# thelovelab/DESeq2

Hardware: AMD Instinct MI355X
Metric: genes/sec for DESeq() disp+beta+Wald fit, 50k x 500 x p=4 (throughput of steps pipelined two deep; one call at a time: one_call_at_a_time) (higher is better)
Workload: dtype f64; 1 GPU; BASELINE configs[2]: 50k genes x 500 samples, ~batch+condition (p=4), Wald; 50000 non-zero genes in total, sharded over 1 GPU(s) in the contiguous ranges of R/parallel.R:10; inputs resident in HBM in R layout (int32 counts, f64 nf matrix; the fused chain reads the size factors as the m-vector the matrix was built from); genes_total=50000, genes_this_gpu=50000, samples=500, p=4, test=Wald, parallelism=gene-shard x1, chain=fused device-driven (dsq_deseq_dev), steps_overlap=step k enqueued while step k-1's results are copied and post-processed

## Files before the change

deseq2_amd/csrc/aux.hip:

```cpp
#include "dsq_internal.hpp"
#include "dsq_math.hpp"
#include "dsq_wave.hpp"

namespace dsq {

static constexpr int kAuxBatch = 4;

static inline int aux_grid_fwd(int n) {
    int blocks = (n + 3) / 4;
    int cap = device_cu_count() * 8;
    return blocks < cap ? (blocks < 1 ? 1 : blocks) : cap;
}

static constexpr int kTileS = 256;
__host__ __device__ static inline bool aux_tiled(int m, int p) { return (size_t)m * p >= 8192 && p <= 24; }

template <int P, bool USE_W, bool TILED>
__global__ void __launch_bounds__(256) prefit_kernel(PrefitKernelParams kp) {
    extern __shared__ __attribute__((aligned(16))) double tile[];
    const int lane = threadIdx.x & 63;
    const int wave = threadIdx.x >> 6;
    const int waves = blockDim.x >> 6;
    const int m = kp.m;
    double rr[P][P];
#pragma unroll
    for (int c = 0; c < P; c++)
#pragma unroll
        for (int k = 0; k < P; k++) rr[c][k] = kp.r[c + P * k];
    const int nwork = DSQ_NWORK(kp);
    for (int wbase = blockIdx.x * waves; wbase < nwork; wbase += gridDim.x * waves) {
        const int wi = wbase + wave;
        const bool active = wi < nwork;
        if (!TILED && !active) break;
        const int g = DSQ_GENE(kp, active ? wi : nwork - 1);
        const int32_t *yg = kp.y + (size_t)g * kp.ld;
        const double *nfg = kp.nf_is_vector ? kp.nf : kp.nf + (size_t)g * kp.ld;
        const double *wg = USE_W ? kp.weights + (size_t)g * kp.ld : nullptr;
        int32_t yb[kAuxBatch];
        double nb[kAuxBatch], wb[kAuxBatch];
        auto load_row = [&](int j, int b) {
            yb[b] = yg[j]; nb[b] = nfg[j];
            if constexpr (USE_W) wb[b] = wg[j];
        };
        double a2[2] = {0.0, 0.0};
        sweep_batched<kAuxBatch>(m, lane, load_row, [&](int, int b) {
            double yy = (double)yb[b];
            double cn = yy / nb[b];
            if constexpr (USE_W) cn = wb[b] * cn;
            a2[0] += cn;
            a2[1] += yy;
        });
        wave_allreduce_many(a2, lane);
        const double mean = a2[0] / (double)m;
        double av = 0.0;
        sweep_batched<kAuxBatch>(m, lane, load_row, [&](int, int b) {
            double cn = (double)yb[b] / nb[b];
            if constexpr (USE_W) cn = wb[b] * cn;
            double dlt = cn - mean;
            av += dlt * dlt;
        });
        av = wave_allreduce(av);
        double tu[2 * P];
#pragma unroll
        for (int c = 0; c < 2 * P; c++) tu[c] = 0.0;
        double ae = 0.0;
        if constexpr (TILED) {
            static_assert(kTileS == 64 * kAuxBatch, "one tile = one batch of trips");
            auto stage = [&](const double *src, int t0) {
                __syncthreads();
                const int ts = (m - t0) < kTileS ? (m - t0) : kTileS;
                for (int idx = threadIdx.x; idx < P * kTileS; idx += blockDim.x) {
                    const int c = idx / kTileS, jj = idx - c * kTileS;
                    if (jj < ts) tile[idx] = src[(size_t)c * m + t0 + jj];
                }
                __syncthreads();
            };
            for (int t0 = 0; t0 < m; t0 += kTileS) {
                stage(kp.q, t0);
                _Pragma("unroll")
                for (int b = 0; b < kAuxBatch; b++) { const int j = t0 + 64 * b + lane; if (j < m) { yb[b] = yg[j]; nb[b] = nfg[j]; } }
                _Pragma("unroll")
                for (int b = 0; b < kAuxBatch; b++) {
                    const int j = t0 + 64 * b + lane;
                    if (j < m) {
                        double yn = (double)yb[b] / nb[b];
                        double ly = dlog(yn + 0.1);
#pragma unroll
                        for (int c = 0; c < P; c++) {
                            double qv = tile[c * kTileS + 64 * b + lane];
// ... 645 lines not shown
hipError_t launch_trend_fit_dev_zeroed(const double *means, const double *disps, const int32_t *n_dev, double *coefs,
                                       int32_t *status, void *workspace, hipStream_t st) {
    hipLaunchKernelGGL(trend_fit_kernel, dim3(kTrendBlocks), dim3(1024), 0, st, means, disps, 0L, n_dev, coefs, status,
                       (TrendWs *)workspace);
    return hipGetLastError();
}

static inline int aux_grid(int n) {
    int blocks = (n + 3) / 4;
    int cap = device_cu_count() * 8;
    return blocks < cap ? (blocks < 1 ? 1 : blocks) : cap;
}

template <int P>
static hipError_t launch_prefit_p(const PrefitKernelParams &kp, hipStream_t st) {
    if constexpr (P <= 24) {
        if (aux_tiled(kp.m, P)) {
            const size_t lds = (size_t)P * kTileS * sizeof(double);
            if (kp.useWeights) hipLaunchKernelGGL((prefit_kernel<P, true, true>), dim3(aux_grid(kp.n)), dim3(256), lds, st, kp);
            else hipLaunchKernelGGL((prefit_kernel<P, false, true>), dim3(aux_grid(kp.n)), dim3(256), lds, st, kp);
            return hipGetLastError();
        }
    }
    if (kp.useWeights) hipLaunchKernelGGL((prefit_kernel<P, true, false>), dim3(aux_grid(kp.n)), dim3(256), 0, st, kp);
    else hipLaunchKernelGGL((prefit_kernel<P, false, false>), dim3(aux_grid(kp.n)), dim3(256), 0, st, kp);
    return hipGetLastError();
}

hipError_t launch_prefit(const PrefitKernelParams &kp, hipStream_t st, bool *ok) {
    *ok = true;
    switch (kp.p) {
#define DSQ_X(W) case W: return launch_prefit_p<W>(kp, st);
    DSQ_P_EACH(DSQ_X)
#undef DSQ_X
    default: *ok = false; return hipSuccess;
    }
}

template <int P>
static hipError_t launch_linear_mu_p(const PrefitKernelParams &kp, double mu_floor, double *mu, hipStream_t st) {
    if constexpr (P <= 24) {
        if (aux_tiled(kp.m, P)) {
            hipLaunchKernelGGL((linear_mu_kernel<P, true>), dim3(aux_grid(kp.n)), dim3(256), (size_t)P * kTileS * sizeof(double), st, kp, mu_floor, mu);
            return hipGetLastError();
        }
    }
// ... 36 lines not shown
```

deseq2_amd/csrc/pipeline.hip:

```cpp
#include "capi.hpp"
#include "dsq_math.hpp"
#include "dsq_wave.hpp"

#include <algorithm>
#include <cstdio>
#include <cstdlib>
#include <cstring>
#include <vector>

namespace dsq {

hipError_t launch_trend_fit_dev(const double *means, const double *disps, const int32_t *n_dev, double *coefs,
                                int32_t *status, void *workspace, hipStream_t st);
hipError_t launch_trend_fit_dev_zeroed(const double *means, const double *disps, const int32_t *n_dev, double *coefs,
                                       int32_t *status, void *workspace, hipStream_t st);
size_t trend_fit_workspace_bytes();

DSQ_DEV double np_min(double a, double b) { return (a != a || b != b) ? a + b : (a < b ? a : b); }
DSQ_DEV double np_max(double a, double b) { return (a != a || b != b) ? a + b : (a > b ? a : b); }

struct Rows {
    const int32_t *rows;
    const int32_t *n_dev;
    int n;
};
DSQ_DEV int rows_count(const Rows &r) { return r.n_dev ? *r.n_dev : r.n; }
DSQ_DEV int rows_gene(const Rows &r, int i) { return r.rows ? r.rows[i] : i; }

__global__ void __launch_bounds__(1024) compact_kernel(int mode, int n, int32_t *allZero, const int32_t *force_zero,
                                                       const double *mean_in, const double *disp_in, double thresh,
                                                       int32_t *rows_out, double *mean_out, double *disp_out,
                                                       int32_t *count_out) {
    constexpr int NT = 4;
    __shared__ int wcnt[NT][16];
    __shared__ int base_s;
    const int t = threadIdx.x, lane = t & 63, wave = t >> 6;
    if (t == 0) base_s = 0;
    __syncthreads();
    for (int i0 = 0; i0 < n; i0 += NT * 1024) {
        bool keep[NT];
        double mv[NT], dv[NT];
#pragma unroll
        for (int q = 0; q < NT; q++) {
            const int i = i0 + q * 1024 + t;
            keep[q] = false; mv[q] = 0.0; dv[q] = 0.0;
            if (i < n) {
                if (mode == 0) {
                    int z = allZero[i] | (force_zero ? force_zero[i] : 0);
                    if (force_zero) allZero[i] = z ? 1 : 0;
                    keep[q] = !z;
                } else {
                    dv[q] = disp_in[i]; mv[q] = mean_in[i];
                    keep[q] = dv[q] > thresh;
                }
            }
        }
        unsigned long long mask[NT];
#pragma unroll
        for (int q = 0; q < NT; q++) {
            mask[q] = __ballot(keep[q]);
            if (lane == 0) wcnt[q][wave] = __popcll(mask[q]);
        }
        __syncthreads();
        int off = base_s;
#pragma unroll
        for (int q = 0; q < NT; q++) {
            int mine = off;
            for (int w = 0; w < 16; w++) { const int c = wcnt[q][w]; if (w < wave) mine += c; off += c; }
            mine += __popcll(mask[q] & ((1ull << lane) - 1ull));
            if (keep[q]) {
                const int i = i0 + q * 1024 + t;
                if (mode == 0) rows_out[mine] = i;
                else { mean_out[mine] = mv[q]; disp_out[mine] = dv[q]; }
            }
        }
        __syncthreads();
        if (t == 0) base_s = off;
        __syncthreads();
    }
    if (t == 0) *count_out = base_s;
}

DSQ_DEV uint64_t key_of(double d) {
    uint64_t u = d2bits(d);
    return (u >> 63) ? ~u : (u | 0x8000000000000000ULL);
}
DSQ_DEV double double_of(uint64_t k) {
    uint64_t u = (k >> 63) ? (k & 0x7fffffffffffffffULL) : ~k;
    return bits2d(u);
}

static constexpr int kSelDirect = 1024;
DSQ_DEV uint64_t rank_direct(const uint64_t *keys, int cnt, long rank, unsigned long long *bc) {
    for (int t = threadIdx.x; t < cnt; t += blockDim.x) {
        const uint64_t mine = keys[t];
        int before = 0;
        for (int j = 0; j < cnt; j++) {
            const uint64_t o = keys[j];
            before += (o < mine || (o == mine && j < t)) ? 1 : 0;
        }
        if (before == (int)rank) bc[0] = mine;
    }
    __syncthreads();
// ... 426 lines not shown
    double minDisp, maxDisp, xim, outlierSD;
    const double *xim_dev;
    int maxit, betaMaxit;
    const double *baseMean, *baseVar, *roughDisp;
    double *alpha_init, *la0;
    const double *la_out, *initial_lp, *last_lp;
    const int32_t *iter;
    const double *la_grid;
    double *dge;
    int32_t *dispGeneIter;
    int32_t *grid_flag, *grid_rows, *grid_count;
    const double *scalars;
    double *dispFit, *log_dfit, *la_init, *dispMAP, *dispersion;
    const double *dispFit_in;
    int32_t *dispIter, *dispOutlier;
    const double *beta_nat, *beta_var, *beta_iter, *logLike;
    double *beta, *betaSE, *stat, *pvalue, *betaIter_out;
    int32_t *betaConv, *optim_flag, *optim_count;
    int32_t *optim_rows;
    int wald;
    const double *beta_init;
    double *opt_start;
    const int32_t *opt_conv;
};

__global__ void alpha_init_kernel(RuleParams q) {
    const int i = blockIdx.x * blockDim.x + threadIdx.x;
    if (i >= rows_count(q.rw)) return;
    const int g = rows_gene(q.rw, i);
    const double bm = q.baseMean[g], bv = q.baseVar[g];
    const double xim = q.xim_dev ? *q.xim_dev : q.xim;
    const double mom = (bv - xim * bm) / (bm * bm);
    double a = np_min(q.roughDisp[g], mom);
    a = np_min(np_max(q.minDisp, a), q.maxDisp);
    q.alpha_init[g] = a;
    q.la0[g] = dlog(a);
}

__global__ void gene_est_post_kernel(RuleParams q) {
    const int i = blockIdx.x * blockDim.x + threadIdx.x;
    if (i >= rows_count(q.rw)) return;
    const int g = rows_gene(q.rw, i);
    double d = np_min(dexp(q.la_out[g]), q.maxDisp);
    const double ilp = q.initial_lp[g];
    if (q.last_lp[g] < ilp + __builtin_fabs(ilp) / 1e6) d = q.alpha_init[g];
    const int it = q.iter[g];
    q.dispGeneIter[g] = it;
    const bool conv = (it < q.maxit) && !(it == 1);
    const bool refit = !conv && (d > q.minDisp * 10.0);
    q.dge[g] = d;
    q.grid_flag[g] = refit ? 1 : 0;
    if (refit) q.grid_rows[atomicAdd(q.grid_count, 1)] = g;
}

__global__ void gene_est_final_kernel(RuleParams q) {
    const int i = blockIdx.x * blockDim.x + threadIdx.x;
    if (i >= rows_count(q.rw)) return;
    const int g = rows_gene(q.rw, i);
    double d = q.dge[g];
    if (q.grid_flag[g]) d = dexp(q.la_grid[g]);
    q.dge[g] = np_min(np_max(d, q.minDisp), q.maxDisp);
}

__global__ void map_init_kernel(RuleParams q) {
    const int i = blockIdx.x * blockDim.x + threadIdx.x;
    if (i >= rows_count(q.rw)) return;
    const int g = rows_gene(q.rw, i);
    const double fit = q.dispFit_in ? q.dispFit_in[g] : q.scalars[DSQ_SC_COEF0] + q.scalars[DSQ_SC_COEF1] / q.baseMean[g];
    const double d = q.dge[g];
    double init = (d > 0.1 * fit) ? d : fit;
    if (init != init) init = fit;
    q.dispFit[g] = fit;
    q.log_dfit[g] = dlog(fit);
    q.la_init[g] = dlog(init);
}

__global__ void map_post_kernel(RuleParams q) {
    const int i = blockIdx.x * blockDim.x + threadIdx.x;
    if (i >= rows_count(q.rw)) return;
    const int g = rows_gene(q.rw, i);
    const int it = q.iter[g];
    q.dispMAP[g] = dexp(q.la_out[g]);
    q.dispIter[g] = it;
    const bool refit = !(it < q.maxit);
    q.grid_flag[g] = refit ? 1 : 0;
    if (refit) q.grid_rows[atomicAdd(q.grid_count, 1)] = g;
}

__global__ void map_final_kernel(RuleParams q) {
    const int i = blockIdx.x * blockDim.x + threadIdx.x;
    if (i >= rows_count(q.rw)) return;
    const int g = rows_gene(q.rw, i);
// ... 48 lines not shown
    }
}

__global__ void optim_post_kernel(RuleParams q) {
    const int cnt = rows_count(q.rw);
    for (int i = blockIdx.x * blockDim.x + threadIdx.x; i < cnt; i += gridDim.x * blockDim.x) {
        const int g = rows_gene(q.rw, i);
        if (q.betaConv && q.opt_conv[g]) q.betaConv[g] = 1;
        if (q.wald && q.stat) {
            for (int c = 0; c < q.p; c++) {
                const double z = q.beta[(size_t)g + (size_t)q.n * c] / q.betaSE[(size_t)g + (size_t)q.n * c];
                q.stat[(size_t)g + (size_t)q.n * c] = z;
                q.pvalue[(size_t)g + (size_t)q.n * c] = dpnorm_upper2(z);
            }
        }
    }
}

__global__ void list_kernel(Rows rw, const int32_t *flag, int want, int32_t *rows_out, int32_t *count) {
    const int i = blockIdx.x * blockDim.x + threadIdx.x;
    if (i >= rows_count(rw)) return;
    const int g = rows_gene(rw, i);
    if ((flag[g] != 0) == (want != 0)) rows_out[atomicAdd(count, 1)] = g;
}

struct NaRowsParams {
    Rows rw;
    int n, p;
    const int32_t *allZero, *n_refit;
    double *beta, *betaSE, *stat, *pvalue, *betaIter, *logLike, *logLikeReduced, *maxCooks;
    int32_t *betaConv;
};
__global__ void na_rows_kernel(NaRowsParams q) {
    const int i = blockIdx.x * blockDim.x + threadIdx.x;
    if (i >= rows_count(q.rw) || *q.n_refit <= 0) return;
    const int g = rows_gene(q.rw, i);
    if (!q.allZero[g]) return;
    const double nan = dnan();
    for (int c = 0; c < q.p; c++) {
        q.beta[(size_t)g + (size_t)q.n * c] = nan;
        q.betaSE[(size_t)g + (size_t)q.n * c] = nan;
        if (q.stat) { q.stat[(size_t)g + (size_t)q.n * c] = nan; q.pvalue[(size_t)g + (size_t)q.n * c] = nan; }
    }
    q.betaIter[g] = nan; q.logLike[g] = nan; q.maxCooks[g] = nan;
    if (q.logLikeReduced) q.logLikeReduced[g] = nan;
    q.betaConv[g] = -1;
// ... 176 lines not shown
    memset(&kp, 0, sizeof kp);
    kp.n = P.n; kp.m = P.m; kp.ld = P.ld;
    kp.y = y; kp.nf = P.a->nf; kp.nf_is_vector = P.a->nf_is_vector;
    kp.weights = P.a->useWeights ? weights : nullptr; kp.useWeights = kp.weights ? 1 : 0;
    kp.rows = rw.rows; kp.n_dev = rw.n_dev;
    return kp;
}

static RuleParams rule_params(const Pipe &P, const Rows &rw) {
    RuleParams q;
    memset(&q, 0, sizeof q);
    const DsqDeseqArgs *a = P.a;
    const DsqDeseqOut *o = P.o;
    q.rw = rw; q.n = P.n; q.p = P.p;
    q.minDisp = a->minDisp; q.maxDisp = P.maxDisp; q.xim = a->xim; q.outlierSD = a->outlierSD;
    q.xim_dev = a->nf_is_vector ? nullptr : P.xim_cur;
    q.maxit = a->maxit; q.betaMaxit = P.t_maxit;
    q.baseMean = o->baseMean; q.baseVar = o->baseVar; q.roughDisp = P.roughDisp;
    q.alpha_init = P.alpha_init; q.la0 = P.la0;
    q.la_out = P.la_out; q.initial_lp = P.initial_lp; q.last_lp = P.last_lp; q.iter = P.iter; q.la_grid = P.la_grid;
    q.dge = o->dispGeneEst; q.dispGeneIter = o->dispGeneIter;
    q.grid_flag = P.grid_flag; q.grid_rows = P.rows_grid;
    q.scalars = o->scalars;
    q.dispFit_in = a->dispFit_in;
    q.dispFit = o->dispFit; q.log_dfit = P.log_dfit; q.la_init = P.la_init; q.dispMAP = o->dispMAP;
    q.dispersion = o->dispersion; q.dispIter = o->dispIter; q.dispOutlier = o->dispOutlier;
    q.beta_nat = P.beta_nat; q.beta_var = P.beta_var; q.beta_iter = P.beta_iter;
    q.optim_rows = P.rows_opt; q.beta_init = P.beta_init; q.opt_start = P.opt_start; q.opt_conv = P.opt_conv;
    return q;
}

enum { DES_FULL = 0, DES_REDUCED = 1, DES_PRIOR = 2 };
struct DesignSel {
    const double *x, *beta_init, *lam;
    int p;
    const int32_t *cperm, *cstart;
    int ncell;
    int p_true;
};
static DesignSel design_of(const Pipe &P, int which) {
    const DsqDeseqArgs *a = P.a;
    DesignSel d;
    if (which == DES_REDUCED) d = {P.red_x_k, P.red_binit, P.red_lam, P.red_pk, P.red_cell_perm, P.red_cell_start, P.red_ncell, a->p_red};
    else if (which == DES_PRIOR) d = {P.pri_x_k, a->prior_expanded ? P.red_binit : P.beta_init, P.lam_prior, P.pri_pk,
                                      P.cell_perm, P.cell_start, P.ncell, a->p_prior};
    else d = {P.x_k, P.beta_init, P.lam, P.pk, P.cell_perm, P.cell_start, P.ncell, P.p};
    return d;
// ... 117 lines not shown
    kp.beta = via_work ? P.opt_beta : beta; kp.betaSE = via_work ? P.opt_se : betaSE;
    kp.conv = P.opt_conv; kp.mu_out = mu_out; kp.loglike = loglike;
    bool ok = false;
    char nm[32];
    snprintf(nm, sizeof nm, "optim_rows%s", P.tag);
    capi_prof_begin(nm, P.n, P.st);
    DSQ_HIP(dispatch_optim_rows(kp.p, kp, P.st, &ok));
    capi_prof_end(P.st);
    if (!ok) return capi_fail(DSQ_ERR_UNSUPPORTED, "dsq_deseq_dev: no optim kernel for p=%d", P.p);
    if (via_work) {
        hipLaunchKernelGGL(copy_rows_cols_kernel, dim3(16), dim3(256), 0, P.st, orw, P.n, ds.p_true, (const double *)P.opt_beta,
                           (const double *)P.opt_se, beta, betaSE);
        DSQ_HIP(hipGetLastError());
    }
    return DSQ_OK;
}

static Rows lpt_rows(Pipe &P, const Rows &rw, const int32_t *key_i, const double *key_d, int small_first = 0) {
    if (!tuning().lpt || rw.rows != P.rows_nz || P.n > tuning().lpt_maxn) return rw;
    hipLaunchKernelGGL(lpt_order_kernel, dim3(1), dim3(1024), 0, P.st, rw, key_i, key_d, small_first, P.rows_lpt);
    return Rows{P.rows_lpt, rw.n_dev, rw.n};
}

static int gene_est(Pipe &P, const Rows &rw, const int32_t *y, double *mu_hat, int cnt_grid, int cnt_optim,
                    int32_t *optim_flag) {
    const DsqDeseqArgs *a = P.a;
    RuleParams q = rule_params(P, rw);
    hipLaunchKernelGGL(alpha_init_kernel, ew_grid(P.n), dim3(256), 0, P.st, q);
    int rc;
    if (a->linearMu) {
        bool ok = false;
        capi_prof_begin("linear_mu", P.n, P.st);
        DSQ_HIP(launch_linear_mu(prefit_params(P, rw, y), P.ge_floor, mu_hat, P.st, &ok));
        capi_prof_end(P.st);
        if (!ok) return capi_fail(DSQ_ERR_UNSUPPORTED, "dsq_deseq_dev: p=%d", P.p);
    } else {
        rc = launch_fit_beta(P, lpt_rows(P, rw, nullptr, P.o->baseMean, 1), y, P.alpha_init, a->weights_norm, mu_hat, P.ge_floor, nullptr,
                             1e-8, 100, 1, 0.5, "fit_beta");
        if (rc) return rc;
        RuleParams b = rule_params(P, rw);
        b.betaMaxit = 100;
        b.optim_flag = optim_flag; b.optim_count = P.counters + cnt_optim;
        hipLaunchKernelGGL(beta_post_kernel, ew_grid(P.n), dim3(256), 0, P.st, b);
        rc = launch_optim(P, cnt_optim, y, P.alpha_init, a->weights_norm, 0.5, P.ge_floor, P.opt_beta, P.opt_se, P.opt_ll, mu_hat);
        if (rc) return rc;
    }
    rc = launch_fit_disp(P, rw, y, mu_hat, P.la0, P.la0, false, a->weights_floor, a->useCR != 0, false, "fit_disp");
    if (rc) return rc;
    q.grid_count = P.counters + cnt_grid;
    hipLaunchKernelGGL(gene_est_post_kernel, ew_grid(P.n), dim3(256), 0, P.st, q);
    Rows gr = {P.rows_grid, P.counters + cnt_grid, P.n};
    rc = launch_fit_disp(P, gr, y, mu_hat, P.la0, P.la0, false, a->weights_floor, a->useCR != 0, true, "fit_disp_grid");
    if (rc) return rc;
    hipLaunchKernelGGL(gene_est_final_kernel, ew_grid(P.n), dim3(256), 0, P.st, q);
    DSQ_HIP(hipGetLastError());
    return DSQ_OK;
}

static int map_est(Pipe &P, const Rows &rw, const int32_t *y, const double *mu_hat, int cnt_grid) {
    const DsqDeseqArgs *a = P.a;
    RuleParams q = rule_params(P, rw);
    hipLaunchKernelGGL(map_init_kernel, ew_grid(P.n), dim3(256), 0, P.st, q);
    int rc = launch_fit_disp(P, rw, y, mu_hat, P.la_init, P.log_dfit, true, a->weights_norm, a->useCR != 0, false, "fit_disp");
    if (rc) return rc;
    q.grid_count = P.counters + cnt_grid;
    hipLaunchKernelGGL(map_post_kernel, ew_grid(P.n), dim3(256), 0, P.st, q);
    Rows gr = {P.rows_grid, P.counters + cnt_grid, P.n};
    rc = launch_fit_disp(P, gr, y, mu_hat, P.la_init, P.log_dfit, true, a->weights_norm, true, true, "fit_disp_grid");
    if (rc) return rc;
    hipLaunchKernelGGL(map_final_kernel, ew_grid(P.n), dim3(256), 0, P.st, q);
    DSQ_HIP(hipGetLastError());
    return DSQ_OK;
}

__global__ void prior_start_kernel(Rows rw, int n, int p, int intercept, const double *bm, double *binit) {
    const int i = blockIdx.x * blockDim.x + threadIdx.x;
    if (i >= rows_count(rw)) return;
    const int g = rows_gene(rw, i);
    for (int c = 0; c < p; c++) binit[(size_t)g + (size_t)n * c] = intercept ? (c == 0 ? dlog(bm[g]) : 0.0) : 1.0;
}

static int mle_fit(Pipe &P, const Rows &rw, const int32_t *y, double *mu_out, double *hat) {
    const DsqDeseqArgs *a = P.a;
    const DsqDeseqOut *o = P.o;
// ... 378 lines not shown
    }
    P.pri_x_k = a->x_prior; P.pri_pk = P.pkp;
    if (a->betaPrior && P.pkp > a->p_prior)
        if ((rc = capi_pad_design(DSQ_WS_PIPE_PADXR, a->x_prior, m, a->p_prior, P.pkp, st, &P.pri_x_k))) return rc;
    if (a->cell_of && a->ncell > 0)
        P.ncell = capi_upload_cells(a->cell_of, m, DSQ_WS_PIPE_CELLS, st, &P.cell_perm, &P.cell_start);
    if (a->x_red || a->betaPrior) {
        if (a->x_red && a->cell_of_red && a->ncell_red > 0)
            P.red_ncell = capi_upload_cells(a->cell_of_red, m, DSQ_WS_PIPE_CELLS_RED, st, &P.red_cell_perm, &P.red_cell_start);
        void *b;
        if ((rc = capi_ws_get(DSQ_WS_PIPE_RED_MU, (size_t)n * P.ld * sizeof(double), &b))) return rc;
        P.red_mu = (double *)b;
    }
    return DSQ_OK;
}

static int xim_scratch(const Pipe &P, double **out) {
    void *b;
    const int rc = capi_ws_get(DSQ_WS_PIPE_XIM_SCRATCH, ((size_t)P.m + 8) * sizeof(double), &b);
    *out = (double *)b;
    return rc;
}

static int phase_gene_est(Pipe &P, const Rows &nz) {
    const DsqDeseqArgs *a = P.a;
    const DsqDeseqOut *o = P.o;
    const Rows all = {nullptr, nullptr, P.n};
    int rc = launch_prefit_rows(P, all, a->y);
    if (rc) return rc;
    hipLaunchKernelGGL(compact_kernel, dim3(1), dim3(1024), 0, P.st, 0, P.n, o->allZero, a->force_zero,
                       (const double *)nullptr, (const double *)nullptr, 0.0, P.rows_nz, (double *)nullptr,
                       (double *)nullptr, P.counters + CNT_NZ);
    if (!a->nf_is_vector) {
        double *b;
        if ((rc = xim_scratch(P, &b))) return rc;
        DSQ_HIP(launch_xim_rows(a->nf, P.rows_nz, P.counters + CNT_NZ, P.m, P.ld, b, P.xim_dev, P.st));
    }
    return gene_est(P, nz, a->y, o->mu_hat, CNT_GRID1, CNT_OPT1, o->optim_geneest);
}

static int phase_trend(Pipe &P) {
    const DsqDeseqArgs *a = P.a;
    const DsqDeseqOut *o = P.o;
    hipStream_t st = P.st;
    const double *tm = a->trend_mean ? a->trend_mean : o->baseMean;
    const double *td = a->trend_mean ? a->trend_disp : o->dispGeneEst;
    const int nt = a->trend_mean ? a->n_trend : P.n;
    if (!(a->phases & DSQ_PH_GENE_EST)) DSQ_HIP(hipMemsetAsync(P.counters + CNT_TREND, 0, sizeof(int32_t), st));
    hipLaunchKernelGGL(compact_kernel, dim3(1), dim3(1024), 0, st, 1, nt, (int32_t *)nullptr, (const int32_t *)nullptr,
                       tm, td, 100.0 * a->minDisp, (int32_t *)nullptr, P.trend_mean_c, P.trend_disp_c,
                       P.counters + CNT_TREND);
    capi_prof_begin("trend_fit", nt, st);
    if (a->dispFit_in) {
        hipLaunchKernelGGL(trend_given_kernel, dim3(1), dim3(1), 0, st, o->scalars, o->status);
    } else {
        if (a->fitType != DSQ_FIT_MEAN)
            DSQ_HIP(launch_trend_fit_dev_zeroed(P.trend_mean_c, P.trend_disp_c, P.counters + CNT_TREND, o->scalars + DSQ_SC_COEF0,
                                                 o->status + DSQ_ST_TREND_STATUS, P.trend_ws, st));
        if (a->fitType != DSQ_FIT_PARAMETRIC)
            hipLaunchKernelGGL(trend_mean_kernel, dim3(1), dim3(1024), 0, st, td, nt, a->minDisp, (int)a->fitType, o->scalars, o->status);
    }
    capi_prof_end(st);
    capi_prof_begin("prior_var", nt, st);
    const double *fin = a->dispFit_in ? (a->trend_mean ? a->trend_fit_in : a->dispFit_in) : (const double *)nullptr;
    if (!P.sel_ws)
        hipLaunchKernelGGL(prior_var_kernel, dim3(1), dim3(1024), 0, st, tm, td, nt, a->minDisp, a->expVarLogDisp,
                           (P.m > P.p) ? 1 : 0, P.resbuf, o->scalars, o->status, fin, a->dispPriorVar_in);
    else
        hipLaunchKernelGGL(prior_var_grid_kernel, dim3(kSelBlocks), dim3(1024), 0, st, tm, td, nt, a->minDisp, a->expVarLogDisp,
                           (P.m > P.p) ? 1 : 0, P.resbuf, o->scalars, o->status, fin, a->dispPriorVar_in, (SelWs *)P.sel_ws);
    capi_prof_end(st);
    DSQ_HIP(hipGetLastError());
    return DSQ_OK;
}

static int phase_map_test(Pipe &P, const Rows &nz, bool *counters_zeroed) {
    const DsqDeseqArgs *a = P.a;
    const DsqDeseqOut *o = P.o;
    if (!(a->phases & DSQ_PH_GENE_EST)) {
        DSQ_HIP(hipMemsetAsync(P.counters + CNT_GRID2, 0, sizeof(int32_t), P.st));
        DSQ_HIP(hipMemsetAsync(P.counters + CNT_OPT2, 0, sizeof(int32_t), P.st));
        DSQ_HIP(hipMemsetAsync(P.counters + CNT_OPT3, 0, sizeof(int32_t), P.st));
    }
    int rc = map_est(P, nz, a->y, o->mu_hat, CNT_GRID2);
    if (rc) return rc;
    if ((rc = test_fit(P, nz, a->y, o->mu, o->H, CNT_OPT2))) return rc;
    const bool z = *counters_zeroed = (a->phases & (DSQ_PH_OUTLIERS | DSQ_PH_OUTLIERS_DETECT)) && !((a->phases & DSQ_PH_PRIOR) && a->betaPrior);
    hipLaunchKernelGGL(na_assay_rows_kernel, ew_grid(P.n), dim3(256), 0, P.st, P.n, P.m, P.ld, (const int32_t *)o->allZero, o->mu, o->H,
                       z ? P.counters + CNT_REP : (int32_t *)nullptr, z ? (int)(CNT_N - CNT_REP) : 0);
    return DSQ_OK;
}

static int phase_prior(Pipe &P, const Rows &nz) {
    DSQ_HIP(hipMemsetAsync(P.counters + CNT_OPT2, 0, sizeof(int32_t), P.st));
    return prior_fit(P, nz, P.a->y, CNT_OPT2);
}

static int phase_outlier_detect(Pipe &P, const Rows &nz, const OutlierMeta &M, bool counters_zeroed) {
    const DsqDeseqArgs *a = P.a;
    const DsqDeseqOut *o = P.o;
    const int n = P.n, m = P.m;
    hipStream_t st = P.st;
    if (!counters_zeroed) DSQ_HIP(hipMemsetAsync(P.counters + CNT_REP, 0, (CNT_N - CNT_REP) * sizeof(int32_t), st));
    CooksKernelParams ck;
    memset(&ck, 0, sizeof ck);
    ck.n = n; ck.m = m; ck.p = P.p; ck.ld = P.ld; ck.y = a->y; ck.nf = a->nf; ck.nf_is_vector = a->nf_is_vector;
    ck.mu = o->mu; ck.H = o->H; ck.perm = M.dperm; ck.cell_start = M.dstart; ck.in3 = M.din3; ck.ncell = a->ncell; ck.any3 = M.any3;
// ... 5 lines not shown
    capi_prof_begin("cooks_distance", n, st);
    DSQ_HIP(launch_cooks(ck, st, &ok));
    capi_prof_end(st);
    if (!ok) return capi_fail(DSQ_ERR_UNSUPPORTED, "m=%d samples: a gene row plus its sort buffer exceeds the 160 KiB LDS", m);
    hipLaunchKernelGGL(na_assay_rows_kernel, ew_grid(n), dim3(256), 0, st, n, m, P.ld, (const int32_t *)o->allZero, o->cooks,
                       (double *)nullptr);
    if (!a->do_replace) return DSQ_OK;
    ReplaceKernelParams rk;
    memset(&rk, 0, sizeof rk);
    rk.n = n; rk.m = m; rk.ld = P.ld; rk.y = a->y; rk.nf = a->nf; rk.nf_is_vector = a->nf_is_vector;
    rk.cooks = o->cooks; rk.cutoff = a->cooksCutoff; rk.trim = a->trim; rk.replaceable = M.drepl;
    int cap2 = 2; while (cap2 < m) cap2 <<= 1;
    rk.sortcap = cap2;
    rk.newCounts = o->replaceCounts; rk.replace = o->replace;
    rk.rows = nz.rows; rk.n_dev = nz.n_dev;
    capi_prof_begin("replace_outliers", n, st);
    DSQ_HIP(launch_replace(rk, st, &ok));
    capi_prof_end(st);
    if (!ok) return capi_fail(DSQ_ERR_UNSUPPORTED, "m=%d samples: the sort buffer exceeds the 160 KiB LDS", m);
    hipLaunchKernelGGL(list_kernel, ew_grid(n), dim3(256), 0, st, nz, (const int32_t *)o->replace, 1, P.rows_rep, P.counters + CNT_REP);
    const Rows rep = {P.rows_rep, P.counters + CNT_REP, n};
    const int rc = launch_prefit_rows(P, rep, o->replaceCounts);
    if (rc) return rc;
    hipLaunchKernelGGL(list_kernel, ew_grid(n), dim3(256), 0, st, rep, (const int32_t *)o->allZero, 0, P.rows_refit, P.counters + CNT_REFIT);
    return DSQ_OK;
}

static void refit_defaults(Pipe &P) {
    P.tag = ":refit";
    P.t_tol = 1e-8; P.t_maxit = 100; P.t_useQR = 1; P.t_minmu = 0.5; P.ge_floor = 0.5;
}

static int phase_outlier_refit(Pipe &P, const Rows &nz, const OutlierMeta &M) {
    const DsqDeseqArgs *a = P.a;
    const DsqDeseqOut *o = P.o;
    const Rows rep = {P.rows_rep, P.counters + CNT_REP, P.n};
    const Rows rf = {P.rows_refit, P.counters + CNT_REFIT, P.n};
    int rc;
    if ((rc = launch_pending_ll(P, true))) return rc;
    refit_defaults(P);
    if (!a->nf_is_vector) {
        double *b;
        if ((rc = xim_scratch(P, &b))) return rc;
        DSQ_HIP(launch_xim_flagged(a->nf, P.n, P.m, P.ld, o->replace, o->allZero, b, P.xim_dev + 1, P.st));
        P.xim_cur = P.xim_dev + 1;
    }
    if ((rc = gene_est(P, rf, o->replaceCounts, o->mu_hat, CNT_GRID1R, CNT_OPT1R, o->optim_geneest))) return rc;
    if ((rc = map_est(P, rf, o->replaceCounts, o->mu_hat, CNT_GRID2R))) return rc;
    if ((rc = join_side(P))) return rc;
    if ((rc = test_fit(P, rf, o->replaceCounts, o->mu_hat, nullptr, CNT_OPT2R))) return rc;
    if (a->betaPrior && (rc = prior_fit(P, rf, o->replaceCounts, CNT_OPT2R))) return rc;
    return a->defer_finish ? DSQ_OK : outlier_finish(P, nz, rep, M, P.counters + CNT_REFIT);
}

static int run_chain(const DsqDeseqArgs *a, const DsqDeseqOut *o, hipStream_t st, Pipe &P) {
    int rc = check_args(a, o);
    if (rc || (rc = capi_check_device()) || (rc = bind(P, a, o, st)) || (rc = launch_init_fills(P)) || (rc = prepare_designs(P))) return rc;
    const Rows nz = {P.rows_nz, P.counters + CNT_NZ, P.n};
    const int ph = a->phases;
    if ((ph & DSQ_PH_GENE_EST) && (rc = phase_gene_est(P, nz))) return rc;
    if ((ph & DSQ_PH_TREND) && (rc = phase_trend(P))) return rc;
    bool counters_zeroed = false;
    if ((ph & DSQ_PH_MAP_TEST) && (rc = phase_map_test(P, nz, &counters_zeroed))) return rc;
    if ((ph & DSQ_PH_PRIOR) && a->betaPrior && (rc = phase_prior(P, nz))) return rc;
    const bool detect = (ph & (DSQ_PH_OUTLIERS | DSQ_PH_OUTLIERS_DETECT)) != 0, refit = (ph & (DSQ_PH_OUTLIERS | DSQ_PH_OUTLIERS_REFIT)) != 0;
    OutlierMeta M;
    if ((detect || refit || ((ph & DSQ_PH_FINISH) && a->do_replace)) && (rc = outlier_meta(a, P.m, st, &M))) return rc;
    if (detect && (rc = phase_outlier_detect(P, nz, M, counters_zeroed))) return rc;
    if (refit && a->do_replace && (rc = phase_outlier_refit(P, nz, M))) return rc;
    if ((ph & DSQ_PH_FINISH) && a->do_replace)
        return outlier_finish(P, nz, Rows{P.rows_rep, P.counters + CNT_REP, P.n}, M, a->n_refit_global ? a->n_refit_global : P.counters + CNT_REFIT);
// ... 29 lines not shown
```

Measured before the change: 5.498 million genes/s.

## Parallelize compaction, fold alpha-init/final into compaction, register-cache prefit rows

Replaces the single-block compaction kernel with a two-pass multi-block count/scatter. For vector size factors, alpha initialisation is folded into the scatter and refit-list kernels, and the gene-estimate final clamp is folded into the trend compaction or the MAP init kernel, which removes separate elementwise launches. Adds a prefit variant for m<=512 that keeps counts and normalised values in registers, replacing repeated global sweeps. This adds kernel variants and extra register pressure, and it changes when dispGeneEst is finalised relative to its readers.

```diff
diff --git a/deseq2_amd/csrc/aux.hip b/deseq2_amd/csrc/aux.hip
--- a/deseq2_amd/csrc/aux.hip
+++ b/deseq2_amd/csrc/aux.hip
@@ -15,8 +15,10 @@
 static constexpr int kTileS = 256;
 __host__ __device__ static inline bool aux_tiled(int m, int p) { return (size_t)m * p >= 8192 && p <= 24; }
 
-template <int P, bool USE_W, bool TILED>
+static constexpr int kPrefitRegTrips = 8;
+template <int P, bool USE_W, bool TILED, int REG = 0>
 __global__ void __launch_bounds__(256) prefit_kernel(PrefitKernelParams kp) {
+    static_assert(!(TILED && REG > 0), "the register path is the untiled kernel's");
     extern __shared__ __attribute__((aligned(16))) double tile[];
     const int lane = threadIdx.x & 63;
     const int wave = threadIdx.x >> 6;
@@ -36,35 +38,104 @@
         const int32_t *yg = kp.y + (size_t)g * kp.ld;
         const double *nfg = kp.nf_is_vector ? kp.nf : kp.nf + (size_t)g * kp.ld;
         const double *wg = USE_W ? kp.weights + (size_t)g * kp.ld : nullptr;
-        int32_t yb[kAuxBatch];
-        double nb[kAuxBatch], wb[kAuxBatch];
-        auto load_row = [&](int j, int b) {
-            yb[b] = yg[j]; nb[b] = nfg[j];
-            if constexpr (USE_W) wb[b] = wg[j];
-        };
         double a2[2] = {0.0, 0.0};
-        sweep_batched<kAuxBatch>(m, lane, load_row, [&](int, int b) {
-            double yy = (double)yb[b];
-            double cn = yy / nb[b];
-            if constexpr (USE_W) cn = wb[b] * cn;
-            a2[0] += cn;
-            a2[1] += yy;
-        });
-        wave_allreduce_many(a2, lane);
-        const double mean = a2[0] / (double)m;
-        double av = 0.0;
-        sweep_batched<kAuxBatch>(m, lane, load_row, [&](int, int b) {
-            double cn = (double)yb[b] / nb[b];
-            if constexpr (USE_W) cn = wb[b] * cn;
-            double dlt = cn - mean;
-            av += dlt * dlt;
-        });
-        av = wave_allreduce(av);
+        double mean, av = 0.0;
+        [[maybe_unused]] double yn_r[REG > 0 ? REG : 1], wyn_r[(REG > 0 && USE_W) ? REG : 1];
+        if constexpr (REG > 0) {
+            int32_t yr[REG];
+            double nr[REG];
+            [[maybe_unused]] double wr[USE_W ? REG : 1];
+#pragma unroll
+            for (int k = 0; k < REG; k++) {
+                const int j = lane + 64 * k;
+                if (j < m) {
+                    yr[k] = yg[j]; nr[k] = nfg[j];
+                    if constexpr (USE_W) wr[k] = wg[j];
+                }
+            }
+#pragma unroll
+            for (int k = 0; k < REG; k++) {
+                const int j = lane + 64 * k;
+                if (j < m) {
+                    const double yy = (double)yr[k];
+                    double cn = yy / nr[k];
+                    yn_r[k] = cn;
+                    if constexpr (USE_W) { cn = wr[k] * cn; wyn_r[k] = cn; }
+                    a2[0] += cn;
+                    a2[1] += yy;
+                }
+            }
+            wave_allreduce_many(a2, lane);
+            mean = a2[0] / (double)m;
+#pragma unroll
+            for (int k = 0; k < REG; k++) {
+                if (lane + 64 * k < m) {
+                    double cn;
+                    if constexpr (USE_W) cn = wyn_r[k]; else cn = yn_r[k];
+                    const double dlt = cn - mean;
+                    av += dlt * dlt;
+                }
+            }
+            av = wave_allreduce(av);
+        } else {
+            int32_t yb[kAuxBatch];
+            double nb[kAuxBatch], wb[kAuxBatch];
+            auto load_row = [&](int j, int b) {
+                yb[b] = yg[j]; nb[b] = nfg[j];
+                if constexpr (USE_W) wb[b] = wg[j];
+            };
+            sweep_batched<kAuxBatch>(m, lane, load_row, [&](int, int b) {
+                double yy = (double)yb[b];
+                double cn = yy / nb[b];
+                if constexpr (USE_W) cn = wb[b] * cn;
+                a2[0] += cn;
+                a2[1] += yy;
+            });
+            wave_allreduce_many(a2, lane);
+            mean = a2[0] / (double)m;
+            sweep_batched<kAuxBatch>(m, lane, load_row, [&](int, int b) {
+                double cn = (double)yb[b] / nb[b];
+                if constexpr (USE_W) cn = wb[b] * cn;
+                double dlt = cn - mean;
+                av += dlt * dlt;
+            });
+            av = wave_allreduce(av);
+        }
         double tu[2 * P];
 #pragma unroll
         for (int c = 0; c < 2 * P; c++) tu[c] = 0.0;
         double ae = 0.0;
-        if constexpr (TILED) {
+        [[maybe_unused]] int32_t yb[kAuxBatch];
+        [[maybe_unused]] double nb[kAuxBatch];
+        if constexpr (REG > 0) {
+#pragma unroll
+            for (int k = 0; k < REG; k++) {
+                const int j = lane + 64 * k;
+                if (j < m) {
+                    const double yn = yn_r[k];
+                    const double ly = dlog(yn + 0.1);
+#pragma unroll
+                    for (int c = 0; c < P; c++) {
+                        const double qv = kp.q[(size_t)c * m + j];
+                        tu[c] += yn * qv;
+                        tu[P + c] += ly * qv;
+                    }
+                }
+            }
+            wave_allreduce_many(tu, lane);
+#pragma unroll
+            for (int k = 0; k < REG; k++) {
+                const int j = lane + 64 * k;
+                if (j < m) {
+                    double mu = tu[0] * kp.a[j];
+#pragma unroll
+                    for (int c = 1; c < P; c++) mu = __builtin_fma(tu[c], kp.a[(size_t)c * m + j], mu);
+                    mu = __builtin_fmax(1.0, mu);
+                    const double d = yn_r[k] - mu;
+                    ae += (d * d - mu) / (mu * mu);
+                }
+            }
+        } else if constexpr (TILED) {
             static_assert(kTileS == 64 * kAuxBatch, "one tile = one batch of trips");
             auto stage = [&](const double *src, int t0) {
                 __syncthreads();
@@ -756,6 +827,13 @@
             return hipGetLastError();
         }
     }
+    if constexpr (P <= DSQ_P_REG) {
+        if (kp.m <= 64 * kPrefitRegTrips) {
+            if (kp.useWeights) hipLaunchKernelGGL((prefit_kernel<P, true, false, kPrefitRegTrips>), dim3(aux_grid(kp.n)), dim3(256), 0, st, kp);
+            else hipLaunchKernelGGL((prefit_kernel<P, false, false, kPrefitRegTrips>), dim3(aux_grid(kp.n)), dim3(256), 0, st, kp);
+            return hipGetLastError();
+        }
+    }
     if (kp.useWeights) hipLaunchKernelGGL((prefit_kernel<P, true, false>), dim3(aux_grid(kp.n)), dim3(256), 0, st, kp);
     else hipLaunchKernelGGL((prefit_kernel<P, false, false>), dim3(aux_grid(kp.n)), dim3(256), 0, st, kp);
     return hipGetLastError();
diff --git a/deseq2_amd/csrc/pipeline.hip b/deseq2_amd/csrc/pipeline.hip
--- a/deseq2_amd/csrc/pipeline.hip
+++ b/deseq2_amd/csrc/pipeline.hip
@@ -27,58 +27,64 @@
 DSQ_DEV int rows_count(const Rows &r) { return r.n_dev ? *r.n_dev : r.n; }
 DSQ_DEV int rows_gene(const Rows &r, int i) { return r.rows ? r.rows[i] : i; }
 
-__global__ void __launch_bounds__(1024) compact_kernel(int mode, int n, int32_t *allZero, const int32_t *force_zero,
-                                                       const double *mean_in, const double *disp_in, double thresh,
-                                                       int32_t *rows_out, double *mean_out, double *disp_out,
-                                                       int32_t *count_out) {
-    constexpr int NT = 4;
-    __shared__ int wcnt[NT][16];
+static constexpr int kCompactTile = 1024;
+static inline int compact_tiles(int n) { return n > 0 ? (n + kCompactTile - 1) / kCompactTile : 1; }
+
+DSQ_DEV bool compact_keep(int mode, int i, const int32_t *allZero, const double *disp_in, double thresh) {
+    return mode == 0 ? allZero[i] == 0 : disp_in[i] > thresh;
+}
+
+template <class Pre>
+DSQ_DEV void compact_count_body(int mode, int n, int32_t *allZero, const int32_t *force_zero, const double *disp_in, double thresh,
+                                int32_t *tile_cnt, Pre &&pre) {
+    const int i = blockIdx.x * kCompactTile + (int)threadIdx.x;
+    bool keep = false;
+    if (i < n) {
+        pre(i);
+        if (mode == 0 && force_zero) allZero[i] = (allZero[i] | force_zero[i]) ? 1 : 0;
+        keep = compact_keep(mode, i, allZero, disp_in, thresh);
+    }
+    const int c = __syncthreads_count(keep ? 1 : 0);
+    if (threadIdx.x == 0) tile_cnt[blockIdx.x] = c;
+}
+__global__ void __launch_bounds__(kCompactTile) compact_count_kernel(int mode, int n, int32_t *allZero, const int32_t *force_zero,
+                                                                     const double *disp_in, double thresh, int32_t *tile_cnt) {
+    compact_count_body(mode, n, allZero, force_zero, disp_in, thresh, tile_cnt, [](int) {});
+}
+
+template <class Post>
+DSQ_DEV void compact_scatter_body(int mode, int n, const int32_t *allZero, const double *mean_in, const double *disp_in, double thresh,
+                                  const int32_t *tile_cnt, int32_t *rows_out, double *mean_out, double *disp_out, int32_t *count_out,
+                                  Post &&post) {
+    __shared__ int wcnt[kCompactTile / 64];
     __shared__ int base_s;
     const int t = threadIdx.x, lane = t & 63, wave = t >> 6;
+    const int i = blockIdx.x * kCompactTile + t;
     if (t == 0) base_s = 0;
     __syncthreads();
-    for (int i0 = 0; i0 < n; i0 += NT * 1024) {
-        bool keep[NT];
-        double mv[NT], dv[NT];
-#pragma unroll
-        for (int q = 0; q < NT; q++) {
-            const int i = i0 + q * 1024 + t;
-            keep[q] = false; mv[q] = 0.0; dv[q] = 0.0;
-            if (i < n) {
-                if (mode == 0) {
-                    int z = allZero[i] | (force_zero ? force_zero[i] : 0);
-                    if (force_zero) allZero[i] = z ? 1 : 0;
-                    keep[q] = !z;
-                } else {
-                    dv[q] = disp_in[i]; mv[q] = mean_in[i];
-                    keep[q] = dv[q] > thresh;
-                }
-            }
-        }
-        unsigned long long mask[NT];
-#pragma unroll
-        for (int q = 0; q < NT; q++) {
-            mask[q] = __ballot(keep[q]);
-            if (lane == 0) wcnt[q][wave] = __popcll(mask[q]);
-        }
-        __syncthreads();
-        int off = base_s;
-#pragma unroll
-        for (int q = 0; q < NT; q++) {
-            int mine = off;
-            for (int w = 0; w < 16; w++) { const int c = wcnt[q][w]; if (w < wave) mine += c; off += c; }
-            mine += __popcll(mask[q] & ((1ull << lane) - 1ull));
-            if (keep[q]) {
-                const int i = i0 + q * 1024 + t;
-                if (mode == 0) rows_out[mine] = i;
-                else { mean_out[mine] = mv[q]; disp_out[mine] = dv[q]; }
-            }
-        }
-        __syncthreads();
-        if (t == 0) base_s = off;
-        __syncthreads();
-    }
-    if (t == 0) *count_out = base_s;
+    int before = 0;
+    for (int k = t; k < (int)blockIdx.x; k += kCompactTile) before += tile_cnt[k];
+    for (int o = 32; o > 0; o >>= 1) before += __shfl_xor(before, o, 64);
+    if (lane == 0 && before) atomicAdd(&base_s, before);
+    const bool keep = i < n && compact_keep(mode, i, allZero, disp_in, thresh);
+    const unsigned long long mask = __ballot(keep);
+    if (lane == 0) wcnt[wave] = __popcll(mask);
+    __syncthreads();
+    int mine = base_s, total = base_s;
+    for (int w = 0; w < kCompactTile / 64; w++) { const int c = wcnt[w]; if (w < wave) mine += c; total += c; }
+    mine += __popcll(mask & ((1ull << lane) - 1ull));
+    if (keep) {
+        if (mode == 0) rows_out[mine] = i;
+        else { mean_out[mine] = mean_in[i]; disp_out[mine] = disp_in[i]; }
+        post(i);
+    }
+    if (t == 0 && blockIdx.x == gridDim.x - 1) *count_out = total;
+}
+__global__ void __launch_bounds__(kCompactTile) compact_scatter_kernel(int mode, int n, const int32_t *allZero, const double *mean_in,
+                                                                       const double *disp_in, double thresh, const int32_t *tile_cnt,
+                                                                       int32_t *rows_out, double *mean_out, double *disp_out,
+                                                                       int32_t *count_out) {
+    compact_scatter_body(mode, n, allZero, mean_in, disp_in, thresh, tile_cnt, rows_out, mean_out, disp_out, count_out, [](int) {});
 }
 
 DSQ_DEV uint64_t key_of(double d) {
@@ -551,12 +557,17 @@
     const double *beta_init;
     double *opt_start;
     const int32_t *opt_conv;
+    int fold_final;
+    const int32_t *allZero;
 };
 
+DSQ_DEV void alpha_init_gene(const RuleParams &q, int g);
 __global__ void alpha_init_kernel(RuleParams q) {
     const int i = blockIdx.x * blockDim.x + threadIdx.x;
     if (i >= rows_count(q.rw)) return;
-    const int g = rows_gene(q.rw, i);
+    alpha_init_gene(q, rows_gene(q.rw, i));
+}
+DSQ_DEV void alpha_init_gene(const RuleParams &q, int g) {
     const double bm = q.baseMean[g], bv = q.baseVar[g];
     const double xim = q.xim_dev ? *q.xim_dev : q.xim;
     const double mom = (bv - xim * bm) / (bm * bm);
@@ -582,13 +593,17 @@
     if (refit) q.grid_rows[atomicAdd(q.grid_count, 1)] = g;
 }
 
+DSQ_DEV double gene_est_final_gene(const RuleParams &q, int g) {
+    double d = q.dge[g];
+    if (q.grid_flag[g]) d = dexp(q.la_grid[g]);
+    d = np_min(np_max(d, q.minDisp), q.maxDisp);
+    q.dge[g] = d;
+    return d;
+}
 __global__ void gene_est_final_kernel(RuleParams q) {
     const int i = blockIdx.x * blockDim.x + threadIdx.x;
     if (i >= rows_count(q.rw)) return;
-    const int g = rows_gene(q.rw, i);
-    double d = q.dge[g];
-    if (q.grid_flag[g]) d = dexp(q.la_grid[g]);
-    q.dge[g] = np_min(np_max(d, q.minDisp), q.maxDisp);
+    gene_est_final_gene(q, rows_gene(q.rw, i));
 }
 
 __global__ void map_init_kernel(RuleParams q) {
@@ -596,7 +611,7 @@
     if (i >= rows_count(q.rw)) return;
     const int g = rows_gene(q.rw, i);
     const double fit = q.dispFit_in ? q.dispFit_in[g] : q.scalars[DSQ_SC_COEF0] + q.scalars[DSQ_SC_COEF1] / q.baseMean[g];
-    const double d = q.dge[g];
+    const double d = q.fold_final ? gene_est_final_gene(q, g) : q.dge[g];
     double init = (d > 0.1 * fit) ? d : fit;
     if (init != init) init = fit;
     q.dispFit[g] = fit;
@@ -691,6 +706,22 @@
     if (i >= rows_count(rw)) return;
     const int g = rows_gene(rw, i);
     if ((flag[g] != 0) == (want != 0)) rows_out[atomicAdd(count, 1)] = g;
+}
+__global__ void list_alpha_init_kernel(Rows rw, const int32_t *flag, int want, int32_t *rows_out, int32_t *count, RuleParams q) {
+    const int i = blockIdx.x * blockDim.x + threadIdx.x;
+    if (i >= rows_count(rw)) return;
+    const int g = rows_gene(rw, i);
+    if ((flag[g] != 0) == (want != 0)) { rows_out[atomicAdd(count, 1)] = g; alpha_init_gene(q, g); }
+}
+
+__global__ void __launch_bounds__(kCompactTile) compact_scatter_alpha_kernel(int n, const int32_t *allZero, const int32_t *tile_cnt,
+                                                                             int32_t *rows_out, int32_t *count_out, RuleParams q) {
+    compact_scatter_body(0, n, allZero, nullptr, nullptr, 0.0, tile_cnt, rows_out, nullptr, nullptr, count_out,
+                         [&](int g) { alpha_init_gene(q, g); });
+}
+__global__ void __launch_bounds__(kCompactTile) compact_count_final_kernel(int n, const double *disp_in, double thresh, int32_t *tile_cnt,
+                                                                           RuleParams q) {
+    compact_count_body(1, n, nullptr, nullptr, disp_in, thresh, tile_cnt, [&](int g) { if (q.allZero[g] == 0) gene_est_final_gene(q, g); });
 }
 
 struct NaRowsParams {
@@ -913,7 +944,7 @@
     q.dge = o->dispGeneEst; q.dispGeneIter = o->dispGeneIter;
     q.grid_flag = P.grid_flag; q.grid_rows = P.rows_grid;
     q.scalars = o->scalars;
-    q.dispFit_in = a->dispFit_in;
+    q.dispFit_in = a->dispFit_in; q.allZero = o->allZero;
     q.dispFit = o->dispFit; q.log_dfit = P.log_dfit; q.la_init = P.la_init; q.dispMAP = o->dispMAP;
     q.dispersion = o->dispersion; q.dispIter = o->dispIter; q.dispOutlier = o->dispOutlier;
     q.beta_nat = P.beta_nat; q.beta_var = P.beta_var; q.beta_iter = P.beta_iter;
@@ -1077,11 +1108,17 @@
     return Rows{P.rows_lpt, rw.n_dev, rw.n};
 }
 
+static bool alpha_in_scatter(const DsqDeseqArgs *a) { return a->nf_is_vector != 0; }
+static bool alpha_in_refit_list(const DsqDeseqArgs *a) { return a->nf_is_vector != 0 && (a->phases & DSQ_PH_OUTLIERS) != 0; }
+static bool final_in_trend(const DsqDeseqArgs *a) {
+    return (a->phases & DSQ_PH_GENE_EST) && (a->phases & DSQ_PH_TREND) && !a->trend_mean;
+}
+
 static int gene_est(Pipe &P, const Rows &rw, const int32_t *y, double *mu_hat, int cnt_grid, int cnt_optim,
-                    int32_t *optim_flag) {
+                    int32_t *optim_flag, bool alpha_done, bool final_elsewhere) {
     const DsqDeseqArgs *a = P.a;
     RuleParams q = rule_params(P, rw);
-    hipLaunchKernelGGL(alpha_init_kernel, ew_grid(P.n), dim3(256), 0, P.st, q);
+    if (!alpha_done) hipLaunchKernelGGL(alpha_init_kernel, ew_grid(P.n), dim3(256), 0, P.st, q);
     int rc;
     if (a->linearMu) {
         bool ok = false;
@@ -1107,14 +1144,15 @@
     Rows gr = {P.rows_grid, P.counters + cnt_grid, P.n};
     rc = launch_fit_disp(P, gr, y, mu_hat, P.la0, P.la0, false, a->weights_floor, a->useCR != 0, true, "fit_disp_grid");
     if (rc) return rc;
-    hipLaunchKernelGGL(gene_est_final_kernel, ew_grid(P.n), dim3(256), 0, P.st, q);
+    if (!final_elsewhere) hipLaunchKernelGGL(gene_est_final_kernel, ew_grid(P.n), dim3(256), 0, P.st, q);
     DSQ_HIP(hipGetLastError());
     return DSQ_OK;
 }
 
-static int map_est(Pipe &P, const Rows &rw, const int32_t *y, const double *mu_hat, int cnt_grid) {
+static int map_est(Pipe &P, const Rows &rw, const int32_t *y, const double *mu_hat, int cnt_grid, bool with_final) {
     const DsqDeseqArgs *a = P.a;
     RuleParams q = rule_params(P, rw);
+    q.fold_final = with_final ? 1 : 0;
     hipLaunchKernelGGL(map_init_kernel, ew_grid(P.n), dim3(256), 0, P.st, q);
     int rc = launch_fit_disp(P, rw, y, mu_hat, P.la_init, P.log_dfit, true, a->weights_norm, a->useCR != 0, false, "fit_disp");
     if (rc) return rc;
@@ -1539,21 +1577,36 @@
     return rc;
 }
 
+static void launch_compact(int mode, int n, int32_t *allZero, const int32_t *force_zero, const double *mean_in, const double *disp_in,
+                           double thresh, int32_t *tile_cnt, int32_t *rows_out, double *mean_out, double *disp_out, int32_t *count_out,
+                           hipStream_t st) {
+    const dim3 grid((unsigned)compact_tiles(n)), block(kCompactTile);
+    hipLaunchKernelGGL(compact_count_kernel, grid, block, 0, st, mode, n, allZero, force_zero, disp_in, thresh, tile_cnt);
+    hipLaunchKernelGGL(compact_scatter_kernel, grid, block, 0, st, mode, n, (const int32_t *)allZero, mean_in, disp_in, thresh,
+                       (const int32_t *)tile_cnt, rows_out, mean_out, disp_out, count_out);
+}
+
 static int phase_gene_est(Pipe &P, const Rows &nz) {
     const DsqDeseqArgs *a = P.a;
     const DsqDeseqOut *o = P.o;
     const Rows all = {nullptr, nullptr, P.n};
     int rc = launch_prefit_rows(P, all, a->y);
     if (rc) return rc;
-    hipLaunchKernelGGL(compact_kernel, dim3(1), dim3(1024), 0, P.st, 0, P.n, o->allZero, a->force_zero,
-                       (const double *)nullptr, (const double *)nullptr, 0.0, P.rows_nz, (double *)nullptr,
-                       (double *)nullptr, P.counters + CNT_NZ);
+    if (alpha_in_scatter(a)) {
+        const dim3 grid((unsigned)compact_tiles(P.n)), block(kCompactTile);
+        hipLaunchKernelGGL(compact_count_kernel, grid, block, 0, P.st, 0, P.n, o->allZero, a->force_zero, (const double *)nullptr, 0.0,
+                           (int32_t *)P.resbuf);
+        hipLaunchKernelGGL(compact_scatter_alpha_kernel, grid, block, 0, P.st, P.n, (const int32_t *)o->allZero,
+                           (const int32_t *)P.resbuf, P.rows_nz, P.counters + CNT_NZ, rule_params(P, nz));
+    } else
+        launch_compact(0, P.n, o->allZero, a->force_zero, nullptr, nullptr, 0.0, (int32_t *)P.resbuf, P.rows_nz, nullptr, nullptr,
+                       P.counters + CNT_NZ, P.st);
     if (!a->nf_is_vector) {
         double *b;
         if ((rc = xim_scratch(P, &b))) return rc;
         DSQ_HIP(launch_xim_rows(a->nf, P.rows_nz, P.counters + CNT_NZ, P.m, P.ld, b, P.xim_dev, P.st));
     }
-    return gene_est(P, nz, a->y, o->mu_hat, CNT_GRID1, CNT_OPT1, o->optim_geneest);
+    return gene_est(P, nz, a->y, o->mu_hat, CNT_GRID1, CNT_OPT1, o->optim_geneest, alpha_in_scatter(a), final_in_trend(a));
 }
 
 static int phase_trend(Pipe &P) {
@@ -1564,9 +1617,15 @@
     const double *td = a->trend_mean ? a->trend_disp : o->dispGeneEst;
     const int nt = a->trend_mean ? a->n_trend : P.n;
     if (!(a->phases & DSQ_PH_GENE_EST)) DSQ_HIP(hipMemsetAsync(P.counters + CNT_TREND, 0, sizeof(int32_t), st));
-    hipLaunchKernelGGL(compact_kernel, dim3(1), dim3(1024), 0, st, 1, nt, (int32_t *)nullptr, (const int32_t *)nullptr,
-                       tm, td, 100.0 * a->minDisp, (int32_t *)nullptr, P.trend_mean_c, P.trend_disp_c,
-                       P.counters + CNT_TREND);
+    if (final_in_trend(a)) {
+        const dim3 grid((unsigned)compact_tiles(nt)), block(kCompactTile);
+        hipLaunchKernelGGL(compact_count_final_kernel, grid, block, 0, st, nt, td, 100.0 * a->minDisp, (int32_t *)P.resbuf,
+                           rule_params(P, Rows{P.rows_nz, P.counters + CNT_NZ, P.n}));
+        hipLaunchKernelGGL(compact_scatter_kernel, grid, block, 0, st, 1, nt, (const int32_t *)nullptr, tm, td, 100.0 * a->minDisp,
+                           (const int32_t *)P.resbuf, (int32_t *)nullptr, P.trend_mean_c, P.trend_disp_c, P.counters + CNT_TREND);
+    } else
+        launch_compact(1, nt, nullptr, nullptr, tm, td, 100.0 * a->minDisp, (int32_t *)P.resbuf, nullptr, P.trend_mean_c, P.trend_disp_c,
+                       P.counters + CNT_TREND, st);
     capi_prof_begin("trend_fit", nt, st);
     if (a->dispFit_in) {
         hipLaunchKernelGGL(trend_given_kernel, dim3(1), dim3(1), 0, st, o->scalars, o->status);
@@ -1599,7 +1658,7 @@
         DSQ_HIP(hipMemsetAsync(P.counters + CNT_OPT2, 0, sizeof(int32_t), P.st));
         DSQ_HIP(hipMemsetAsync(P.counters + CNT_OPT3, 0, sizeof(int32_t), P.st));
     }
-    int rc = map_est(P, nz, a->y, o->mu_hat, CNT_GRID2);
+    int rc = map_est(P, nz, a->y, o->mu_hat, CNT_GRID2, false);
     if (rc) return rc;
     if ((rc = test_fit(P, nz, a->y, o->mu, o->H, CNT_OPT2))) return rc;
     const bool z = *counters_zeroed = (a->phases & (DSQ_PH_OUTLIERS | DSQ_PH_OUTLIERS_DETECT)) && !((a->phases & DSQ_PH_PRIOR) && a->betaPrior);
@@ -1651,7 +1710,11 @@
     const Rows rep = {P.rows_rep, P.counters + CNT_REP, n};
     const int rc = launch_prefit_rows(P, rep, o->replaceCounts);
     if (rc) return rc;
-    hipLaunchKernelGGL(list_kernel, ew_grid(n), dim3(256), 0, st, rep, (const int32_t *)o->allZero, 0, P.rows_refit, P.counters + CNT_REFIT);
+    if (alpha_in_refit_list(a)) {
+        hipLaunchKernelGGL(list_alpha_init_kernel, ew_grid(n), dim3(256), 0, st, rep, (const int32_t *)o->allZero, 0, P.rows_refit,
+                           P.counters + CNT_REFIT, rule_params(P, Rows{P.rows_refit, P.counters + CNT_REFIT, n}));
+    } else
+        hipLaunchKernelGGL(list_kernel, ew_grid(n), dim3(256), 0, st, rep, (const int32_t *)o->allZero, 0, P.rows_refit, P.counters + CNT_REFIT);
     return DSQ_OK;
 }
 
@@ -1674,8 +1737,8 @@
         DSQ_HIP(launch_xim_flagged(a->nf, P.n, P.m, P.ld, o->replace, o->allZero, b, P.xim_dev + 1, P.st));
         P.xim_cur = P.xim_dev + 1;
     }
-    if ((rc = gene_est(P, rf, o->replaceCounts, o->mu_hat, CNT_GRID1R, CNT_OPT1R, o->optim_geneest))) return rc;
-    if ((rc = map_est(P, rf, o->replaceCounts, o->mu_hat, CNT_GRID2R))) return rc;
+    if ((rc = gene_est(P, rf, o->replaceCounts, o->mu_hat, CNT_GRID1R, CNT_OPT1R, o->optim_geneest, alpha_in_refit_list(a), true))) return rc;
+    if ((rc = map_est(P, rf, o->replaceCounts, o->mu_hat, CNT_GRID2R, true))) return rc;
     if ((rc = join_side(P))) return rc;
     if ((rc = test_fit(P, rf, o->replaceCounts, o->mu_hat, nullptr, CNT_OPT2R))) return rc;
     if (a->betaPrior && (rc = prior_fit(P, rf, o->replaceCounts, CNT_OPT2R))) return rc;
```

After: 5.578 million genes/s, median of 6. 1.5% higher.
